# DARYL-GWZ/Proud-SLAM

Measured on AMD Instinct MI355X. Metric: rays/sec render+backward, Replica room0, 64 samples/ray, 1/2/4/8 MI355X, higher is better.
Workload: dtype f32

## Files before the change

include/psvo.h:

```cpp
#ifndef PSVO_H
#define PSVO_H

#include <stdint.h>

#ifdef __cplusplus
extern "C" {
#endif

enum {
    PSVO_OK = 0,
    PSVO_E_INVALID = 1,
    PSVO_E_LAUNCH = 2,
    PSVO_E_OVERFLOW = 3,
    PSVO_E_BUSY = 4,
    PSVO_E_SYSTEM = 5
};

const char *psvo_last_error(void);
const char *psvo_version(void);


int psvo_svo_intersect(void *stream, int b, int n, int m, float voxelsize, int n_max, const float *ray_start,
                       const float *ray_dir, const float *points, const int *children, int *idx, float *min_depth,
                       float *max_depth);
// ... 226 lines not shown
                       float *out_dirs, float *out_rgb, float *out_depth);

int64_t psvo_rows_workspace_ints(int64_t n_rows);
int psvo_rows_compact(void *stream, int64_t n_rows, int width, const float *grad, int *workspace, int *ids,
                      float *rows, int *count);
int psvo_rows_scatter_add(void *stream, int64_t n_list, int width, const int *ids, const float *rows, float *grad);
int psvo_rows_compact_flagged(void *stream, int64_t n_rows, int width, const float *grad, const uint8_t *flags,
                              int *workspace, int *ids, float *rows, int *count);
int psvo_rows_clear(void *stream, int64_t n_list, int width, const int *ids, float *grad, uint8_t *flags);
int psvo_rows_mark(void *stream, int64_t n_list, const int *ids, uint8_t *flags);
int psvo_rows_flags_from_grad(void *stream, int64_t n_rows, int width, const float *grad, uint8_t *flags);

psvo_engine *psvo_engine_new(void);
void psvo_engine_free(psvo_engine *e);
enum { PSVO_XCH_GATHER_I32 = 1, PSVO_XCH_SUM_I32 = 2, PSVO_XCH_SUM_F64 = 3, PSVO_XCH_QUERY = 0x100 };
typedef int (*psvo_exchange_fn)(void *user, int op, int64_t in_off, int64_t out_off, int64_t count, void *stream);
int64_t psvo_engine_exchange_words(int world, int64_t max_rays_global, int64_t max_rays_rank);
int psvo_engine_set_exchange(psvo_engine *e, int rank, int world, int64_t max_rays_global, int64_t max_rays_rank,
                             psvo_exchange_fn fn, void *user, int *xi32, double *xf64);

int psvo_engine_queued(psvo_engine *e);
int psvo_map_discard(psvo_engine *e);

enum { PSVO_PATH_QUERY_SPLIT = 1, PSVO_PATH_PADDED = 2, PSVO_PATH_DENSE_DECODER = 4, PSVO_PATH_INTERP_PASS = 8 };
int psvo_engine_set_paths(psvo_engine *e, int paths);

int psvo_engine_select_stats(psvo_engine *e, void *stream, int64_t *out, int reset);

int psvo_engine_gate_stream(psvo_engine *e, void *stream);

int psvo_debug_set_lookback(int mask, int spin_bound, int delay_us);
int psvo_debug_lb_helps(int64_t *out3, int reset);
int psvo_debug_set_pixel_draw(int mode);
int psvo_debug_select_samples(void *stream, int64_t r_hit, int s_max, float truncation, float max_depth,
                              const int *offsets, const int *ray_ns, const float *z_vals, int z_stride,
                              const int *rank_ray, const float *gt_depth, const float *sdf_s, const float *feat,
                              const int *leaf, const float *t, const int *ray_of, int64_t cap, int split, int *cidx,
                              int *offa, int *offb, float *feat_c, int *leaf_c, float *t_c, int *ray_of_c,
                              float *rgb_c, int *src_c, int *counts, uint64_t *desc, uint32_t tag, int *host_flag);
int64_t psvo_debug_select_granules(int64_t r_hit);
int psvo_debug_trunk_interp(void *stream, int fused, int64_t m_cap, const int *m_dev, const int *leaf, const float *t,
                            const int *ray_of, const int *ray_index, const float *rays_o, const float *rays_d,
                            const float *centres, const int *vertex_idx, const float *emb, float voxel_size,
                            const float *w1, const float *b1, const float *w2, const float *b2, const float *w3,
                            const float *b3, const float *w4, const float *b4, const float *w5, const float *b5,
                            float *images, float *sdf, float *h2, float *feat);
int psvo_debug_composite_loss(void *stream, int64_t r_hit, int s_max, float truncation, float max_depth,
                              const int *offsets, const int *ray_ns, const float *z_vals, int z_stride,
                              const int *rank_ray, const float *gt_rgb, const float *gt_depth, const float *sdf_s,
                              const float *rgb_s, const float *coef, float *workspace, float *color, float *depth,
                              float *grad_sdf_s, float *grad_rgb_s, int partials, const int *cidx);

enum { PSVO_TIME_MLP_FWD = 0, PSVO_TIME_MLP_BWD = 1, PSVO_TIME_INTERP_FWD = 2, PSVO_TIME_INTERP_BWD = 3,
       PSVO_TIME_INTERSECT = 4, PSVO_TIME_SAMPLE = 5, PSVO_TIME_POINTS = 6, PSVO_TIME_SELECT = 7,
// ... 130 lines not shown
```

proud-slam_amd/csrc/capi.cpp:

```cpp
#include <hip/hip_runtime.h>
#include <stdarg.h>
#include <stdio.h>

#include "psvo_common.h"
#include "lookback.h"

namespace psvo {

static thread_local char g_err[512] = "";
thread_local hipEvent_t g_stop_event = nullptr;
thread_local bool g_stop_share = false;
thread_local hipEvent_t g_stop_bound = nullptr;

int set_error(int code, const char *fmt, ...) {
    va_list ap;
    va_start(ap, fmt);
    vsnprintf(g_err, sizeof(g_err), fmt, ap);
    va_end(ap);
    return code;
}

int check_launch(const char *what) {
    const hipError_t e = hipGetLastError();
    if (e != hipSuccess) return set_error(PSVO_E_LAUNCH, "%s: %s", what, hipGetErrorString(e));
    return PSVO_OK;
}

static int g_lb_debug_mask = 0, g_lb_debug_bound = -1, g_lb_debug_delay = 0;
LbCtl lb_ctl(int site) {
    const bool on = (g_lb_debug_mask & site) != 0;
    return LbCtl{on && g_lb_debug_bound >= 0 ? g_lb_debug_bound : kLbSpinMax, on ? g_lb_debug_delay : 0};
}

}

extern "C" int psvo_debug_set_lookback(int mask, int spin_bound, int delay_us) {
    PSVO_REQUIRE(mask >= 0 && mask <= 7 && spin_bound >= -1 && delay_us >= 0 && delay_us <= 100000,
                 "debug_set_lookback: bad arguments");
    psvo::g_lb_debug_mask = mask;
    psvo::g_lb_debug_bound = spin_bound;
    psvo::g_lb_debug_delay = delay_us;
    return PSVO_OK;
}

extern "C" int psvo_debug_lb_helps(int64_t *out3, int reset) {
    PSVO_REQUIRE(out3, "debug_lb_helps: null argument");
    const int rc = psvo::lb_helps_query(out3, reset != 0);
    if (rc != PSVO_OK) return rc;
    return psvo::lb_helps_select(out3 + 2, reset != 0);
}

extern "C" int psvo_debug_select_samples(void *stream, int64_t r_hit, int s_max, float truncation, float max_depth,
                                         const int *offsets, const int *ray_ns, const float *z_vals, int z_stride,
                                         const int *rank_ray, const float *gt_depth, const float *sdf_s,
                                         const float *feat, const int *leaf, const float *t, const int *ray_of,
                                         int64_t cap, int split, int *cidx, int *offa, int *offb, float *feat_c,
// ... 25 lines not shown
```

proud-slam_amd/csrc/engine.cpp:

```cpp
#include <stdio.h>
#include <stdlib.h>
#include <string.h>

#include <utility>

#include "engine_internal.h"

namespace psvo {
RenderWs *&engine_render_ws(psvo_engine *e) { return e->render; }
bool engine_data_parallel(const psvo_engine *e) { return e->x.on(); }
}

using namespace psvo;
using namespace psvo::eng;

namespace psvo {
thread_local KernelClock *g_kclock = nullptr;

namespace eng {

void *arena_buf(Arena &a, hipStream_t st, int slot, size_t bytes, int *rc) {
    if (bytes == 0) bytes = 16;
    if (a.cap[slot] >= bytes) return a.p[slot];
    if (a.p[slot]) {
// ... 201 lines not shown
}

int pose_adam(hipStream_t st, const psvo_map_desc *d, const PoseAdam &pa) {
    if (pa.n == 0) return PSVO_OK;
    int64_t n6[kXchMaxFrames];
    double lr[kXchMaxFrames];
    int zero[kXchMaxFrames];
    for (int k = 0; k < pa.n; ++k) {
        n6[k] = 6;
        lr[k] = pa.lr;
        zero[k] = 0;
    }
    return adam_launch(st, pa.n, pa.p, pa.g, pa.m, pa.v, n6, lr, d->beta1, d->beta2, d->eps, 0.0, 1, zero,
                       const_cast<int64_t *>(pa.step));
}

}
}

extern "C" psvo_engine *psvo_engine_new(void) {
    psvo_engine *e = new psvo_engine();
    const char *ipass = getenv("PSVO_INTERP_PASS");
    if (ipass && ipass[0] == '1') e->paths |= PSVO_PATH_INTERP_PASS;
    for (auto &q : e->qs)
        if (query_set_init(q) != PSVO_OK) {
            psvo_engine_free(e);
            return nullptr;
        }
    return e;
}

static EngineExchange exchange_layout(int world, int64_t max_rays_global, int64_t max_rays_rank) {
    EngineExchange x;
    x.world = world;
    x.nch = dist_slot0_rows(max_rays_global) / kSamplerG;
    x.max_rays_rank = max_rays_rank > 0 ? max_rays_rank : max_rays_global;
    x.cw = dist_count_words((int)x.max_rays_rank);
    return x;
}

extern "C" int64_t psvo_engine_exchange_words(int world, int64_t max_rays_global, int64_t max_rays_rank) {
    if (world < 1 || max_rays_global < 1 || max_rays_rank < 0 || max_rays_rank > max_rays_global) return -1;
    const EngineExchange x = exchange_layout(world, max_rays_global, max_rays_rank);
    return x.table_off() + x.table_words();
}

extern "C" int psvo_engine_set_exchange(psvo_engine *e, int rank, int world, int64_t max_rays_global,
                                        int64_t max_rays_rank, psvo_exchange_fn fn, void *user, int *xi32,
                                        double *xf64) {
    PSVO_REQUIRE(e, "engine_set_exchange: null engine");
    PSVO_REQUIRE(world >= 1 && rank >= 0 && rank < world && max_rays_global >= 1 && max_rays_rank >= 0 &&
                     max_rays_rank <= max_rays_global,
                 "engine_set_exchange: bad rank %d / world %d / max_rays_global %lld / max_rays_rank %lld", rank,
                 world, (long long)max_rays_global, (long long)max_rays_rank);
    PSVO_REQUIRE(e->q_count == 0, "engine_set_exchange: queries are queued");
    PSVO_REQUIRE(!fn || (xi32 && xf64), "engine_set_exchange: exchange buffers required");
    e->x = exchange_layout(world, max_rays_global, max_rays_rank);
    e->x.fn = fn;
    e->x.user = user;
    e->x.rank = rank;
    e->x.xi32 = xi32;
    e->x.xf64 = xf64;
    return PSVO_OK;
}

extern "C" int psvo_engine_set_paths(psvo_engine *e, int paths) {
    PSVO_REQUIRE(e && (paths & ~(PSVO_PATH_QUERY_SPLIT | PSVO_PATH_PADDED | PSVO_PATH_DENSE_DECODER |
                               PSVO_PATH_INTERP_PASS)) == 0,
                 "engine_set_paths: bad arguments");
    PSVO_REQUIRE(e->q_count == 0, "engine_set_paths: queries are queued");
    e->paths = paths;
    return PSVO_OK;
}

extern "C" int psvo_engine_gate_stream(psvo_engine *e, void *stream) {
    PSVO_REQUIRE(e, "engine_gate_stream: null engine");
    e->draw_gate_used = true;
    if (!e->draw_gate_recorded) return PSVO_OK;
    return st_wait(as_stream(stream), e->draw_gate_ev, "engine_gate_stream");
}

extern "C" int psvo_engine_select_stats(psvo_engine *e, void *stream, int64_t *out, int reset) {
    PSVO_REQUIRE(e && out, "engine_select_stats: null argument");
    for (int i = 0; i < 5; ++i) out[i] = 0;
    if (!e->a.p[kSelCnt]) return PSVO_OK;
    hipStream_t st = as_stream(stream);
    int c[psvo::kSelCountInts];
    if (hipMemcpyAsync(c, e->a.p[kSelCnt], sizeof(c), hipMemcpyDeviceToHost, st) != hipSuccess ||
        hipStreamSynchronize(st) != hipSuccess)
        return set_error(PSVO_E_LAUNCH, "engine_select_stats: copy failed");
    unsigned long long u[3];
// ... 174 lines not shown
```

proud-slam_amd/csrc/engine_step.cpp:

```cpp
#include <stdint.h>
#include <string.h>

#include <algorithm>

#include "engine_internal.h"
#include "interp_load.h"

using namespace psvo;
using namespace psvo::eng;

namespace {

struct Samples {
    int *offsets = nullptr, *leaf = nullptr, *ray_of = nullptr;
    float *tt = nullptr, *feat = nullptr, *rgb_s = nullptr, *act = nullptr;
    uint64_t *masks = nullptr;
};

struct Render {
    int64_t r_hit = 0, m = 0;
    int s_max = 0;
    int *rank_ray = nullptr, *ray_rank = nullptr, *ray_ns = nullptr;
    float *z_vals = nullptr, *images = nullptr, *sdf_s = nullptr;
    Samples s;
// ... 592 lines not shown
    const Render &q = s.q;
    const Samples &k = s.k;
    int rc = PSVO_OK;
    const int64_t M = q.m, R = s.R;
    const int n_split = 256;
    ENG_BUF(float, mlp_ws, kMlpWs, psvo_mlp_workspace_floats_w(M, d->width, n_split) * sizeof(float));
    ENG_BUF(float, dfeat, kDfeat, M * 16 * sizeof(float));
    const bool fuse_ib = psvo::mlp_bwd_fuses_interp(d->width);
    float *grad_emb = s.grads;
    const size_t emb_bytes = (size_t)d->n_emb * 16 * sizeof(float);
    const bool emb_dirty = !(e->grads_clean && e->clean_buf == grad_emb);
    if (fuse_ib && emb_dirty) ENG_CALL(zero_async(grad_emb, emb_bytes, st, "map_step"));
    float *gx = nullptr;
    if (fuse_ib) {
        ENG_BUF(float, gxb, kIbWs, (size_t)s.m_rows() * 3 * sizeof(float));
        gx = gxb;
    }
    const psvo::InterpFuse ipf{k.leaf,  k.ray_of,      q.rank_ray, d->vertex_idx, k.tt, s.rays_o, s.rays_d, d->centres,
                               d->emb,  d->voxel_size, grad_emb,   gx,            s.mark_into};
    mark(e, st, PSVO_TIME_MLP_BWD, 0);
    const psvo::InterpFuse ipf_b{k.leaf + M, k.ray_of + M, q.rank_ray, d->vertex_idx, k.tt + M, s.rays_o, s.rays_d,
                                 d->centres, d->emb, d->voxel_size, grad_emb, gx ? gx + 3 * M : nullptr, s.mark_into};
    const psvo::TrunkBwd tbw{s.sel_cnt ? s.sel_cnt + 1 : nullptr, s.g_sdf_s + M, s.h2_src ? k.feat : k.feat + M * 16,
                             fuse_ib ? &ipf_b : nullptr, s.h2_src ? q.h2 : nullptr, s.h2_src ? s.h2_src + M : nullptr};
    ENG_CALL(mlp_bwd(st, M, d->width, k.feat, q.images, k.rgb_s, k.act, k.masks, s.g_sdf_s, s.g_rgb_s, dfeat, s.G, 0,
                     n_split, mlp_ws, s.overlap ? e->dfeat_ready : nullptr, fuse_ib ? &ipf : nullptr,
                     s.split ? ax : nullptr, s.sel_cnt, s.two_class() ? &tbw : nullptr, s.h2_src));
    mark(e, st, PSVO_TIME_MLP_BWD, 1);
    if (s.overlap) e->bwd_recorded = true;
    if (s.overlap && eb != st) ENG_CALL(st_wait(eb, e->dfeat_ready, "map_step"));
    if (!fuse_ib && emb_dirty) ENG_CALL(zero_async(grad_emb, emb_bytes, eb, "map_step"));
    e->grads_clean = false;
    e->clean_buf = grad_emb;
    mark(e, eb, PSVO_TIME_INTERP_BWD, 0);
    if (fuse_ib) {
        ENG_CALL(psvo::interp_rays_gx(eb, q.r_hit, k.offsets, q.rank_ray, k.tt, gx, s.grad_od, s.grad_od + R * 3,
                                      s.two_class() ? s.offb : nullptr, s.two_class() ? k.tt + M : nullptr,
                                      s.two_class() ? gx + 3 * M : nullptr));
    } else {
        ENG_BUF(float, ib_ws2, kIbWs, psvo_interp_bwd_workspace_floats(q.r_hit, q.s_max) * sizeof(float));
        ENG_CALL(psvo_interp_bwd_chunked(eb, q.r_hit, q.s_max, 16, d->voxel_size, k.offsets, q.rank_ray, k.leaf, k.tt,
                                         s.rays_o, s.rays_d, d->centres, d->vertex_idx, d->emb, dfeat, grad_emb,
                                         s.grad_od, s.grad_od + R * 3, ib_ws2));
    }
    mark(e, eb, PSVO_TIME_INTERP_BWD, 1);
    if (s.overlap && eb != st) {
        ENG_CALL(ev_record(e->emb_done, eb, "map_step"));
// ... 201 lines not shown
```

proud-slam_amd/csrc/mlp128_trunk_fb.h:

```cpp
#pragma once
#include "interp_fuse.h"
#include "mlp128_chain16.h"

namespace psvo {
namespace {

using ifuse::interp_bwd_unit;
using ifuse::scatter_unit;

constexpr int kT4H2 = kVecPad;
constexpr int kT4H1 = kT4H2 + 4 * kUImg;
constexpr int kT4CF = kT4H1 + 4 * kUImg;
constexpr int kT4X = kT4CF + 2 * kCfTile;
constexpr int kT4I = kT4X + 2 * 4 * 16 * kU;
constexpr int kT4R = kT4I + 4 * 512;
constexpr int kT4M = kT4R + 4 * 132;
constexpr int kLdsTrunk = (kT4M + 4 * 64 * 2) * 4;
static_assert(kLdsTrunk <= 160 * 1024, "trunk kernel LDS budget");

struct TrunkIn {
    float gs;
    float4 x;
    int src;
};
// ... 66 lines not shown
        for (int ob = 0; ob < 8; ++ob)
#pragma unroll
            for (int j = 0; j < 4; ++j) r0[ob][j] = row_sum16(fb[ob][j] * dsdf);
        if (n == 0) {
#pragma unroll
            for (int ob = 0; ob < 8; ++ob) {
                float4 *pp = reinterpret_cast<float4 *>(page3 + 16 * ob + 4 * q);
                const float4 o = *pp;
                *pp = make_float4(o.x + r0[ob][0], o.y + r0[ob][1], o.z + r0[ob][2], o.w + r0[ob][3]);
            }
        }
    }
    b30p += dsdf;
#pragma unroll
    for (int ob = 0; ob < 8; ++ob) {
        const float4 w = *reinterpret_cast<const float4 *>(lds + kOffW3r0 + 16 * ob + 4 * q);
        fb[ob] = f32x4v{__fmul_rn(w.x, dsdf), __fmul_rn(w.y, dsdf), __fmul_rn(w.z, dsdf), __fmul_rn(w.w, dsdf)};
    }
    mask16(fb, m2);
    lds_u_store<8>(lds + kT4H2 + k * kUImg, wb, fb);
}

template <bool H2>
__global__ __launch_bounds__(kF2Threads, 1) void k_mlp_trunk_fb(const int *__restrict__ m_dev,
                                                                const float *__restrict__ img,
                                                                const float *__restrict__ g_sdf,
                                                                const float *__restrict__ feat, DwGrid g,
                                                                float *__restrict__ slabs, InterpFuse ip,
                                                                const float *__restrict__ h2,
                                                                const int *__restrict__ h2_src) {
    extern __shared__ __attribute__((aligned(16))) float lds[];
    const int64_t m = __builtin_amdgcn_readfirstlane(*m_dev);
    const int lane = threadIdx.x & 63;
    const int wave = __builtin_amdgcn_readfirstlane(threadIdx.x >> 6);
    const int64_t n_units = (m + kU - 1) / kU;
    const int64_t u0 = n_units * blockIdx.x / gridDim.x, u1 = n_units * (blockIdx.x + 1) / gridDim.x;
    const int n_rounds = (int)((u1 - u0 + 3) / 4);
    float *const h2set = lds + kT4H2, *const h1set = lds + kT4H1, *const cf = lds + kT4CF;
    auto xset = [&](int par) { return lds + kT4X + (par & 1) * 4 * 16 * kU; };
    stage8(lds, img + kImgVec, kVecPad, wave, lane);
    wait_vm(0);
    raw_barrier();
    const int b = blockIdx.x;
    const int i = lane & 31, h = lane >> 5;
    const int n = lane & 15, q = lane >> 4;
    const int sn = (n & 1) * 8 + (n >> 1);
    const int wb = 64 * q + ((((sn >> 2) ^ q) << 2) | (sn & 3));
    const __amdgpu_buffer_rsrc_t wrs = rsrc_of(img, (int64_t)kImgTotal * 4);
    const bool fuse = ip.gx != nullptr;
    [[maybe_unused]] constexpr int kStampK = 2;
    PSVO_STAMP_DECL;
    if (wave < 4) {
        const int c = wave;
        f32x4v w1acc[8];
        zero4(w1acc);
        float b1p[8] = {0.f, 0.f, 0.f, 0.f, 0.f, 0.f, 0.f, 0.f};
        int lf_n = 0, ro_n = 0;
        float ts_n = 0.f;
        {
            const int64_t u = u0 + c;
            const int64_t s = u * kU + n;
            if (fuse && u < u1 && s < m) {
                lf_n = ip.leaf[s];
                ro_n = ip.ray_of[s];
                ts_n = ip.t[s];
            }
// ... 164 lines not shown
                for (int k = 0; k < 4; ++k) v += lds[kT4M + k * 128 + e - 128 * 16];
            }
            store_nt(s1, e, v);
        }
    }
    if (wave >= 4) {
        const int d = wave - 4;
        float *s3 = slabs + g.slab_off[2] + (int64_t)b * g.slab_len[2];
        if (h == 0) {
            float v = 0.f;
#pragma unroll
            for (int k = 0; k < 4; ++k) v += lds[kT4R + k * 132 + 32 * d + i];
            store_nt(s3, 32 * d + i, v);
        }
        if (d == 0 && lane == 0) {
            float v = 0.f;
#pragma unroll
            for (int k = 0; k < 4; ++k) v += lds[kT4R + k * 132 + 128];
            store_nt(s3, 129 * 128, v);
        }
    }
}

void launch_trunk_fb(hipStream_t st, int grid, const float *images, const TrunkBwd &tb, const DwGrid &g,
                     float *slabs) {
    const InterpFuse ip = tb.ip ? *tb.ip : InterpFuse{};
    if (tb.h2)
        launch_lds<k_mlp_trunk_fb<true>>(dim3(grid), dim3(kF2Threads), kLdsTrunk, st, tb.m_dev, images, tb.g_sdf,
                                         tb.feat, g, slabs, ip, tb.h2, tb.src);
    else
        launch_lds<k_mlp_trunk_fb<false>>(dim3(grid), dim3(kF2Threads), kLdsTrunk, st, tb.m_dev, images, tb.g_sdf,
                                          tb.feat, g, slabs, ip, tb.h2, tb.src);
}

}
}
```

proud-slam_amd/csrc/mlp_bwd.hip:

```cpp
#include <hip/hip_runtime.h>

#include <cstdlib>

#include "interp_fuse.h"
#include "mlp128_chain16.h"
#include "mlp128_trunk_fb.h"
#include "psvo_common.h"

namespace psvo {
namespace {

constexpr int kDwRedEl = 64;
__device__ __forceinline__ float dw_sum_range(const float *__restrict__ p, int64_t stride, int b, int e) {
    float v = 0.0f;
    int sp = b;
    for (; sp + 8 <= e; sp += 8) {
        float q[8];
#pragma unroll
        for (int u = 0; u < 8; ++u) q[u] = p[(sp + u) * stride];
#pragma unroll
        for (int u = 0; u < 8; ++u) v += q[u];
    }
    for (; sp < e; ++sp) v += p[sp * stride];
    return v;
}
__global__ __launch_bounds__(256) void k_mlp_dw_reduce(DwGrid g, const float *__restrict__ slabs, DwDst dst,
                                                       int accumulate, const float *__restrict__ slabs_b) {
    __shared__ float part[4][kDwRedEl];
    const int lane = threadIdx.x & 63, k = threadIdx.x >> 6;
    const int e = blockIdx.x * kDwRedEl + lane;
    const bool in = e < dst.elem_begin[5];
    int L = 0;
#pragma unroll
    for (int l = 1; l < 5; ++l) L += (e >= dst.elem_begin[l]);
    const int rel = in ? e - dst.elem_begin[L] : 0;
    const int n_split = g.n_split[L];
    const int64_t stride = g.slab_len[L];
    const int b = n_split * k / 4, en = n_split * (k + 1) / 4;
    float v = 0.0f;
    if (in) {
        v = dw_sum_range(slabs + g.slab_off[L] + rel, stride, b, en);
        if (slabs_b && (L < 2 || (L == 2 && (rel < 128 || rel == 129 * 128))))
            v += dw_sum_range(slabs_b + g.slab_off[L] + rel, stride, b, en);
    }
    part[k][lane] = v;
    __syncthreads();
    if (k != 0 || !in) return;
    v = ((part[0][lane] + part[1][lane]) + part[2][lane]) + part[3][lane];
    const int nw = dst.rows[L] * dst.cols[L];
    float *out = rel < nw ? dst.w[L] + rel : dst.b[L] + (rel - nw);
    *out = accumulate ? *out + v : v;
}

struct BwdIn16 {
    uint64_t mk[3];
    float y[3], g[3], gs;
    float4 x;
};

__device__ __forceinline__ void load_bwd_in16(const float *__restrict__ rgb_in, const uint64_t *__restrict__ masks,
                                              const float *__restrict__ g_sdf, const float *__restrict__ g_rgb,
                                              const float *__restrict__ feat, int64_t s, bool valid, int q,
                                              BwdIn16 &in, const int *__restrict__ x_src = nullptr) {
    const int64_t sv = valid ? s : 0;
    const uint64_t *mk = masks + (sv * 2 + (q & 1)) * 3;
#pragma unroll
    for (int i = 0; i < 3; ++i) {
        in.mk[i] = mk[i];
        in.y[i] = rgb_in[sv * 3 + i];
        in.g[i] = g_rgb[sv * 3 + i];
    }
    in.gs = g_sdf[sv];
    const int64_t xr = x_src ? (int64_t)x_src[sv] : sv;
    in.x = *reinterpret_cast<const float4 *>(feat + xr * kIn + 4 * q);
}

struct Bwd3Src {
    const float *rgb, *g_sdf, *g_rgb, *feat;
    const uint64_t *masks;
    const float *act;
    float *dfeat;
    const int *x_src;
};

template <bool W>
__global__ __launch_bounds__(kF2Threads, 1) void k_mlp_bwd3(int64_t m, const float *__restrict__ img, Bwd3Src src,
                                                            DwGrid g, float *__restrict__ slabs, InterpFuse ip,
                                                            const int *__restrict__ m_dev) {
    extern __shared__ __attribute__((aligned(16))) float lds[];
    if (m_dev) m = __builtin_amdgcn_readfirstlane(*m_dev);
    const int lane = threadIdx.x & 63;
    const int wave = __builtin_amdgcn_readfirstlane(threadIdx.x >> 6);
    const int64_t n_tiles = (m + kCh - 1) / kCh * 2;
    const int64_t tstride = n_tiles * kCfTile;
    const int64_t tb = tstride * 4;
    const int64_t n_units = (m + kU - 1) / kU;
    const int64_t u0 = n_units * blockIdx.x / gridDim.x, u1 = n_units * (blockIdx.x + 1) / gridDim.x;
    constexpr int kPer = W ? 4 : 8;
    const int n_rounds = (int)((u1 - u0 + kPer - 1) / kPer);
    float *const slot = lds + kB3Slot, *const small = lds + kB3Small, *const xim = lds + kB3X;
    auto dset = [&](int s) { return slot + s * 4 * kUImg; };
    auto eset = [&](int e) { return dset(((e % 2) + 2) % 2); };
    auto sset = [&](int s) { return small + s * 4 * 4 * kU; };
    auto xset = [&](int par) { return xim + par * 4 * 16 * kU; };
    stage8(lds, img + kImgVec, kVecPad, wave, lane);
    wait_vm(0);
    raw_barrier();
    const int b = blockIdx.x;
    const int i = lane & 31, h = lane >> 5;
    if (!W || wave < 4) {
        const __amdgpu_buffer_rsrc_t wrs = rsrc_of(img, (int64_t)kImgTotal * 4);
        const int c = wave;
        const int n = lane & 15, q = lane >> 4;
        const int sn = (n & 1) * 8 + (n >> 1);
        const int wb = 64 * q + ((((sn >> 2) ^ q) << 2) | (sn & 3));
        float *const page1 = lds + kB3A + c * 2048, *const page4x = page1 + 1024;
        if (W) {
#pragma unroll
            for (int k = 0; k < 8; ++k)
                *reinterpret_cast<float4 *>(page1 + (k * 64 + lane) * 4) = make_float4(0.f, 0.f, 0.f, 0.f);
        }
        float b1p = 0.f;
        BwdIn16 nin;
        {
            const int64_t u = u0 + c;
            const int64_t s = u * kU + n;
            load_bwd_in16(src.rgb, src.masks, src.g_sdf, src.g_rgb, src.feat, s, u < u1 && s < m, q, nin, src.x_src);
        }
        [[maybe_unused]] constexpr int kStampK = 1;
        PSVO_STAMP_DECL;
        for (int r = 0; r <= n_rounds; ++r) {
// ... 238 lines not shown
            store_nt(s3, 32 * d + i, vr0);
        }
        if (d == 0 && lane == 0) store_nt(s3, 129 * 128, v30);
        float *s5 = slabs + g.slab_off[4] + (int64_t)b * g.slab_len[4];
        const float4 p0 = *reinterpret_cast<const float4 *>(page5), p1 = *reinterpret_cast<const float4 *>(page5 + 4);
        const float w5[3] = {p0.x, p0.y, p0.z}, b5[3] = {p1.x, p1.y, p1.z};
        float v5[3], t5[3];
#pragma unroll
        for (int ch = 0; ch < 3; ++ch) {
            v5[ch] = w5[ch] + __shfl_xor(w5[ch], 32, 64);
            t5[ch] = b5[ch] + __shfl_xor(b5[ch], 32, 64);
        }
        if (h == 0) {
#pragma unroll
            for (int ch = 0; ch < 3; ++ch) store_nt(s5, ch * 128 + 32 * d + i, v5[ch]);
        }
        if (d == 0 && lane == 0) {
#pragma unroll
            for (int ch = 0; ch < 3; ++ch) store_nt(s5, 3 * 128 + ch, t5[ch]);
        }
    }
}

int bwd3_grid(int64_t m) {
    const int64_t rounds = (m + 4 * kU - 1) / (4 * kU);
    return persistent_grid(rounds > 0 ? rounds : 1);
}
constexpr int kDwRows[5] = {128, 128, 129, 128, 3};
constexpr int kDwCols[5] = {16, 128, 128, 144, 128};
void dw_grid_uniform(int n, DwGrid *g, int *slab_floats) {
    int off = 0;
    for (int l = 0; l < 5; ++l) {
        g->n_split[l] = n;
        g->slab_off[l] = off;
        g->slab_len[l] = kDwRows[l] * kDwCols[l] + kDwRows[l];
        off += n * g->slab_len[l];
    }
    *slab_floats = off;
}

}

int64_t dec128_workspace_floats(int64_t m) {
    DwGrid g;
    int slab;
    dw_grid_uniform(bwd3_grid(m), &g, &slab);
    return m * 3 + 2 * (int64_t)slab;
}

int dec128_bwd(hipStream_t st, int64_t m, const float *feat, const float *images, const float *rgb, const float *act,
               const uint64_t *masks, const float *g_sdf, const float *g_rgb, float *dfeat, float *const gw[5],
               float *const gb[5], int accumulate, int n_split, float *workspace, hipEvent_t dfeat_ready,
               const InterpFuse *ip, hipStream_t reduce_stream, const int *m_dev, const TrunkBwd *tb,
               const int *x_src) {
    PSVO_REQUIRE(m >= 0 && n_split > 0, "mlp_bwd: bad sizes");
    PSVO_REQUIRE(images != nullptr, "mlp_bwd: images of the training forward required");
    const bool want_w = gw[0] != nullptr;
    PSVO_REQUIRE(!want_w || act != nullptr, "mlp_bwd: weight gradients need the forward's activations");
    DwGrid g;
    int slab_floats;
    PSVO_REQUIRE(tb == nullptr || (gw[0] != nullptr && tb->m_dev && tb->g_sdf && tb->feat),
                 "mlp_bwd: the trunk backward needs the weight-gradient path and its inputs");
    float *slabs_b = nullptr;
    auto reduce = [&](float *slabs, hipStream_t rs) {
        DwDst d;
        int e = 0;
        for (int l = 0; l < 5; ++l) {
            d.w[l] = gw[l];
            d.b[l] = gb[l];
            d.rows[l] = kDwRows[l];
            d.cols[l] = kDwCols[l];
            d.elem_begin[l] = e;
            e += kDwRows[l] * kDwCols[l] + kDwRows[l];
        }
        d.elem_begin[5] = e;
        psvo::launch(k_mlp_dw_reduce, dim3(div_up(e, kDwRedEl)), dim3(256), 0, rs, g, slabs, d, accumulate,
                     static_cast<const float *>(slabs_b));
        return check_launch("mlp_dw_reduce");
    };
    Bwd3Src src{rgb, g_sdf, g_rgb, feat, masks, act, dfeat, x_src};
    if (!want_w) {
        if (m > 0) {
            launch_lds<k_mlp_bwd3<false>>(dim3(persistent_grid(div_up(div_up(m, kU), 8))), dim3(kF2Threads), kLdsBwd3,
                                          st, m, images, src, g, nullptr, InterpFuse{}, m_dev);
            const int rc = check_launch("mlp_bwd3");
            if (rc) return rc;
        }
        if (dfeat_ready && hipEventRecord(dfeat_ready, st) != hipSuccess)
            return set_error(PSVO_E_LAUNCH, "mlp_bwd: event record failed");
        return PSVO_OK;
    }
    const int grid = bwd3_grid(m);
    dw_grid_uniform(grid, &g, &slab_floats);
    float *slabs = workspace + m * 3;
    static const bool bind_env = [] {
        const char *v = getenv("PSVO_BIND_DFEAT");
        return !(v && v[0] == '0');
    }();
    const bool trunk_last = tb && m > 0;
    bool bound = false;
    const hipEvent_t bind_ev = bind_env ? dfeat_ready : nullptr;
    if (m > 0) {
        psvo::StopBind sb(trunk_last ? nullptr : bind_ev);
        launch_lds<k_mlp_bwd3<true>>(dim3(grid), dim3(kF2Threads), kLdsBwd3, st, m, images, src, g, slabs,
                                     ip ? *ip : InterpFuse{}, m_dev);
        bound = sb.consumed();
        const int rc = check_launch("mlp_bwd3");
        if (rc) return rc;
    } else if (hipMemsetAsync(slabs, 0, (size_t)slab_floats * sizeof(float), st) != hipSuccess) {
        return set_error(PSVO_E_LAUNCH, "mlp_bwd: memset failed");
    }
    if (trunk_last) {
        slabs_b = slabs + slab_floats;
        PSVO_REQUIRE(!tb->h2 || tb->src, "mlp_bwd: the trunk's h2 rows need their source index");
        psvo::StopBind sb(bind_ev);
        launch_trunk_fb(st, grid, images, *tb, g, slabs_b);
        bound = sb.consumed();
        const int rc = check_launch("mlp_trunk_fb");
        if (rc) return rc;
    }
    if (dfeat_ready && !bound && hipEventRecord(dfeat_ready, st) != hipSuccess)
        return set_error(PSVO_E_LAUNCH, "mlp_bwd: event record failed");
    if (reduce_stream && reduce_stream != st) {
        PSVO_REQUIRE(dfeat_ready != nullptr, "mlp_bwd: a separate reduce stream needs the dfeat_ready event");
        if (hipStreamWaitEvent(reduce_stream, dfeat_ready, 0) != hipSuccess)
            return set_error(PSVO_E_LAUNCH, "mlp_bwd: stream wait failed");
        return reduce(slabs, reduce_stream);
    }
    return reduce(slabs, st);
}

}
```

proud-slam_amd/csrc/psvo_common.h:

```cpp
#pragma once

#include <hip/hip_ext.h>
#include <hip/hip_runtime.h>
#include <stdint.h>

#include "../../include/psvo.h"

namespace psvo {

struct KernelClock {
    static constexpr int kMax = 192, kMaxInst = 64;
    hipEvent_t ev[kMax][2] = {};
    int region[kMax] = {};
    int n = 0;
    struct Inst {
        int region, first, last;
    } inst[kMaxInst] = {};
    int n_inst = 0;
    int stack[8] = {};
    int depth = 0;
    bool sum = false;
    bool overflow = false;
    hipStream_t streams[4] = {};
    bool owns(hipStream_t st) const {
// ... 293 lines not shown
    coef[2] = (flags & PSVO_CRIT_USE_SDF) ? (float)(2.0 * (double)(fs_w * fs_weight) / n_el) : 0.0f;
    coef[3] = (flags & PSVO_CRIT_USE_SDF) ? (float)(2.0 * (double)(sdf_w * sdf_weight) / n_el) * tr : 0.0f;
}

struct InterpFuse {
    const int *leaf, *ray_of, *rank_ray, *vertex_idx;
    const float *t, *rays_o, *rays_d, *centres, *emb;
    float voxel_size;
    float *grad_emb;
    float *gx;
    uint8_t *row_flags;
};

int interp_rays_gx(hipStream_t st, int64_t r_hit, const int *offsets, const int *ray_index, const float *t,
                   const float *gx, float *grad_o, float *grad_d, const int *offsets2 = nullptr,
                   const float *t2 = nullptr, const float *gx2 = nullptr);

struct TrunkBwd {
    const int *m_dev;
    const float *g_sdf, *feat;
    const InterpFuse *ip;
    const float *h2 = nullptr;
    const int *src = nullptr;
};
int mlp_bwd(void *stream, int64_t m, int width, const float *feat, const float *images, const float *rgb,
            const float *act, const uint64_t *masks, const float *g_sdf, const float *g_rgb, float *dfeat,
            float *const *grads, int accumulate, int n_split, float *workspace, hipEvent_t dfeat_ready,
            const InterpFuse *ip = nullptr, hipStream_t reduce_stream = nullptr, const int *m_dev = nullptr,
            const TrunkBwd *tb = nullptr,
            const int *x_src = nullptr);
bool mlp_bwd_fuses_interp(int width);
bool mlp_bwd_split_tail(int width);

int mlp_images(void *stream, int width, const float *const *dec, float *images);
struct H2Rows {
    float *out = nullptr;
    const float *rows = nullptr;
    const int *src = nullptr;
};
int mlp_fwd_prepared(void *stream, int64_t m, int width, const float *feat, float *images, float *sdf, float *rgb,
                     float *act, uint64_t *masks, const int *m_dev = nullptr,
                     const H2Rows *h2 = nullptr);
int mlp_fwd(void *stream, int64_t m, int width, const float *feat, const float *const *dec, float *images, float *sdf,
            float *rgb, float *act, uint64_t *masks);

}

// ... 5 lines not shown
```

proud-slam_amd/psvo/_lib.py:

```python
from __future__ import annotations

import ctypes
import os

import torch

PKG_ROOT = os.path.dirname(os.path.dirname(os.path.abspath(__file__)))
LIB_PATH = os.environ.get("PSVO_LIB_PATH") or os.path.join(PKG_ROOT, "lib", "libpsvo.so")

_vp, _i32, _i64, _f32, _f64, _u64 = (ctypes.c_void_p, ctypes.c_int, ctypes.c_int64, ctypes.c_float,
                                      ctypes.c_double, ctypes.c_uint64)

_SIGNATURES = {
    "psvo_last_error": (ctypes.c_char_p, []),
    "psvo_version": (ctypes.c_char_p, []),
    "psvo_svo_intersect": (_i32, [_vp, _i32, _i32, _i32, _f32, _i32] + [_vp] * 7),
    "psvo_inverse_cdf_sampling": (_i32, [_vp, _i32, _i32, _i32, _i32, _f32] + [_vp] * 9),
    "psvo_ball_intersect": (_i32, [_vp, _i32, _i32, _i32, _f32, _i32] + [_vp] * 6),
    "psvo_aabb_intersect": (_i32, [_vp, _i32, _i32, _i32, _f32, _i32] + [_vp] * 6),
    "psvo_triangle_intersect": (_i32, [_vp, _i32, _i32, _i32, _f32, _f32, _i32] + [_vp] * 6),
    "psvo_uniform_ray_sampling": (_i32, [_vp, _i32, _i32, _i32, _i32, _f32] + [_vp] * 7),
    "psvo_ray_intersect_sorted": (_i32, [_vp, _i64, _vp, _vp, _vp, _vp, _f32, _f32, _f32] + [_vp] * 6),
    "psvo_hit_rank": (_i32, [_vp, _i64, _vp, _vp, _vp]),
    "psvo_sample_rays": (_i32, [_vp, _i64, _i32, _vp, _vp, _vp, _vp, _vp, _f32, _vp, _u64, _vp, _vp, _vp, _vp,
# ... 28 lines not shown
    "psvo_rows_mark": (_i32, [_vp, _i64, _vp, _vp]),
    "psvo_rows_flags_from_grad": (_i32, [_vp, _i64, _i32, _vp, _vp]),
    "psvo_mlp_image_floats": (_i64, []),
    "psvo_mlp_image_floats_w": (_i64, [_i32]),
    "psvo_mlp_act_floats": (_i64, [_i64, _i32]),
    "psvo_mlp_mask_words": (_i64, [_i64, _i32]),
    "psvo_mlp_workspace_floats_w": (_i64, [_i64, _i32, _i32]),
    "psvo_map_grad_floats_w": (_i64, [_i64, _i32]),
    "psvo_mlp_fwd": (_i32, [_vp, _i64, _i32] + [_vp] * 16),
    "psvo_mlp_workspace_floats": (_i64, [_i64, _i32]),
    "psvo_mlp_bwd": (_i32, [_vp, _i64, _i32] + [_vp] * 28 + [_i32, _i32, _vp]),
    "psvo_criterion_workspace_floats": (_i64, [_i64]),
    "psvo_criterion_sums": (_i32, [_vp, _i64, _i32, _i32, _f32, _f32] + [_vp] * 9),
    "psvo_criterion_finalize": (_i32, [_vp, _vp, _i64, _i32, _f32, _f32, _f32, _f32, _f32, _i32, _vp]),
    "psvo_criterion_bwd": (_i32, [_vp, _i64, _i32, _f32, _f32] + [_vp] * 12),
    "psvo_adam_step": (_i32, [_vp, _i32, _vp, _vp, _vp, _vp, _vp, _f64, _f64, _f64, _f64, _f64, _i64]),
    "psvo_engine_new": (_vp, []),
    "psvo_engine_free": (None, [_vp]),
    "psvo_engine_set_timing": (_i32, [_vp, _i32]),
    "psvo_engine_set_paths": (_i32, [_vp, _i32]),
    "psvo_engine_select_stats": (_i32, [_vp, _vp, _vp, _i32]),
    "psvo_engine_gate_stream": (_i32, [_vp, _vp]),
    "psvo_debug_set_lookback": (_i32, [_i32, _i32, _i32]),
    "psvo_debug_set_pixel_draw": (_i32, [_i32]),
    "psvo_debug_lb_helps": (_i32, [_vp, _i32]),
    "psvo_debug_select_samples": (_i32, [_vp, _i64, _i32, _f32, _f32, _vp, _vp, _vp, _i32] + [_vp] * 7
                                  + [_i64, _i32] + [_vp] * 11 + [ctypes.c_uint32, _vp]),
    "psvo_debug_select_granules": (_i64, [_i64]),
    "psvo_debug_trunk_interp": (_i32, [_vp, _i32, _i64] + [_vp] * 10 + [_f32] + [_vp] * 14),
    "psvo_debug_composite_loss": (_i32, [_vp, _i64, _i32, _f32, _f32, _vp, _vp, _vp, _i32] + [_vp] * 11
                                  + [_i32, _vp]),
    "psvo_engine_queued": (_i32, [_vp]),
    "psvo_map_discard": (_i32, [_vp]),
    "psvo_engine_exchange_words": (_i64, [_i32, _i64, _i64]),
    "psvo_engine_set_exchange": (_i32, [_vp, _i32, _i32, _i64, _i64, _vp, _vp, _vp, _vp]),
    "psvo_engine_timing": (_i32, [_vp, _vp]),
    "psvo_engine_set_clock": (_i32, [_vp, _i32]),
    "psvo_engine_clock": (_i32, [_vp, _vp, _vp]),
    "psvo_host_wait_stats": (_i32, [_vp, _vp, _vp, _i32]),
    "psvo_map_step": (_i32, [_vp, _vp, _vp, _i64, _vp, _vp, _vp, _vp, _u64, _i64, _i32, _vp, _vp]),
    "psvo_map_adam": (_i32, [_vp, _vp, _vp, _i64]),
    "psvo_map_adam_ex": (_i32, [_vp, _vp, _vp, _i64, _i32]),
    "psvo_map_join": (_i32, [_vp, _vp]),
    "psvo_map_side_wait": (_i32, [_vp, _vp]),
    "psvo_engine_grad_rays": (_i32, [_vp, _vp, _i64, _vp, _vp]),
    "psvo_map_query": (_i32, [_vp, _vp, _vp, _i64, _vp, _vp, _u64]),
# ... 132 lines not shown
```

proud-slam_amd/psvo/engine.py:

```python
from __future__ import annotations

import ctypes
import os

import torch

from . import _lib as L

_vp, _i32, _i64, _f32, _f64 = ctypes.c_void_p, ctypes.c_int, ctypes.c_int64, ctypes.c_float, ctypes.c_double


class MapDesc(ctypes.Structure):
    _fields_ = [("n_nodes", _i64), ("centres", _vp), ("structure", _vp), ("vertex_idx", _vp),
                ("emb", _vp), ("n_emb", _i64), ("emb_m", _vp), ("emb_v", _vp),
                ("dec", _vp * 10), ("dec_m", _vp * 10), ("dec_v", _vp * 10), ("width", _i32),
                ("voxel_size", _f32), ("step_size", _f32), ("max_distance", _f32), ("truncation", _f32),
                ("max_depth", _f32), ("w_rgb", _f32), ("w_depth", _f32), ("w_fs", _f32), ("w_sdf", _f32),
                ("lr_emb", _f64), ("lr_dec", _f64), ("beta1", _f64), ("beta2", _f64), ("eps", _f64),
                ("grad_flat", _vp), ("packed", _vp), ("emb_row_flags", _vp), ("emb_row_local", _vp)]


class MapFrames(ctypes.Structure):
    _fields_ = [("n_frames", _i32), ("rays_per_frame", _i64), ("dirs_cam", _vp), ("poses", _vp), ("pose_m", _vp),
                ("pose_v", _vp), ("pose_step", _vp), ("lr_pose", _f64), ("pose_grad", _vp),
# ... 253 lines not shown
                                   "(pass the same tensor objects and seed)")
        else:
            ro = rays_o.reshape(-1, 3).float().contiguous()
            rd = rays_d.reshape(-1, 3).float().contiguous()
        gt_rgb = rgb.reshape(-1, 3).float().contiguous()
        gt_d = depth.reshape(-1).float().contiguous()
        self.step_no += 1
        rc = _lib().psvo_map_step(self.handle, L.stream_of(ro.device), ctypes.addressof(self.desc), ro.shape[0],
                                  ro.data_ptr(), rd.data_ptr(), gt_rgb.data_ptr(), gt_d.data_ptr(), int(seed),
                                  self.step_no, 0 if apply_adam else 1, self.loss_out.data_ptr(),
                                  ctypes.addressof(self.stats))
        self._sync_queue()
        if rc != 0:
            self.step_no -= 1
            raise self._error("psvo_map_step", rc)
        return self.loss_out[0]

    def adam(self):
        ge = self.grad_exchange
        marked = ge is not None and ge.take_rows_marked()
        L.call("psvo_map_adam_ex", self.handle, L.stream_of(self.emb.device), ctypes.addressof(self.desc),
               self.step_no, 1 if marked else 0)

    PATH_QUERY_SPLIT, PATH_PADDED, PATH_DENSE_DECODER, PATH_INTERP_PASS = 1, 2, 4, 8

    def set_paths(self, paths):
        L.call("psvo_engine_set_paths", self.handle, int(paths))

    def select_stats(self, reset=False):
        out = (ctypes.c_int64 * 5)()
        L.call("psvo_engine_select_stats", self.handle, L.stream_of(self.emb.device), ctypes.cast(out, ctypes.c_void_p),
               int(bool(reset)))
        return {"kept": out[0], "composited": out[1], "kept_sum": out[2], "composited_sum": out[3], "steps": out[4]}

    def set_timing(self, on):
        L.call("psvo_engine_set_timing", self.handle, 2 if on == "overlap" else int(bool(on)))

    def set_clock(self, max_steps):
        L.call("psvo_engine_set_clock", self.handle, int(max_steps))

    def clock(self):
        ms, n = ctypes.c_double(), ctypes.c_int()
        L.call("psvo_engine_clock", self.handle, ctypes.byref(ms), ctypes.byref(n))
        return (ms.value if ms.value >= 0 else None), n.value

    @staticmethod
    def host_wait_stats(reset=False):
# ... 124 lines not shown
```

Measured before the change: 6.323 million.

## Fuse head and trunk MLP backward into one launch with cost-balanced workgroup split

Runs the head-class bwd3 and the trunk backward in a single persistent launch. Workgroups are partitioned between the two classes by a cost model (bwd_split_na) that balances the estimated rounds of each, using device-side counts. This removes a serial kernel boundary and the tail idle time between the two launches. The dw reduce kernel is adjusted to match the new split of slabs. The trade-offs are higher LDS use per workgroup (the max of both kernels' needs) and dependence on hand-tuned cost constants. The old two-launch path stays available behind an env flag.

```diff
diff --git a/include/psvo.h b/include/psvo.h
--- a/include/psvo.h
+++ b/include/psvo.h
@@ -272,7 +272,13 @@
 int psvo_engine_queued(psvo_engine *e);
 int psvo_map_discard(psvo_engine *e);
 
-enum { PSVO_PATH_QUERY_SPLIT = 1, PSVO_PATH_PADDED = 2, PSVO_PATH_DENSE_DECODER = 4, PSVO_PATH_INTERP_PASS = 8 };
+enum {
+    PSVO_PATH_QUERY_SPLIT = 1,
+    PSVO_PATH_PADDED = 2,
+    PSVO_PATH_DENSE_DECODER = 4,
+    PSVO_PATH_INTERP_PASS = 8,
+    PSVO_PATH_BWD_TWO_LAUNCH = 16
+};
 int psvo_engine_set_paths(psvo_engine *e, int paths);
 
 int psvo_engine_select_stats(psvo_engine *e, void *stream, int64_t *out, int reset);
@@ -280,6 +286,8 @@
 int psvo_engine_gate_stream(psvo_engine *e, void *stream);
 
 int psvo_debug_set_lookback(int mask, int spin_bound, int delay_us);
+int psvo_debug_set_bwd_split(int cost_a, int cost_b, int cost_b0);
+int psvo_debug_bwd_split(int64_t units_a, int64_t units_b, int n_wg);
 int psvo_debug_lb_helps(int64_t *out3, int reset);
 int psvo_debug_set_pixel_draw(int mode);
 int psvo_debug_select_samples(void *stream, int64_t r_hit, int s_max, float truncation, float max_depth,
diff --git a/proud-slam_amd/csrc/capi.cpp b/proud-slam_amd/csrc/capi.cpp
--- a/proud-slam_amd/csrc/capi.cpp
+++ b/proud-slam_amd/csrc/capi.cpp
@@ -32,6 +32,25 @@
     return LbCtl{on && g_lb_debug_bound >= 0 ? g_lb_debug_bound : kLbSpinMax, on ? g_lb_debug_delay : 0};
 }
 
+static BwdSplitCost g_bwd_split_cost = kBwdSplitCost;
+BwdSplitCost bwd_split_cost() { return g_bwd_split_cost; }
+
+}
+
+extern "C" int psvo_debug_set_bwd_split(int cost_a, int cost_b, int cost_b0) {
+    if (cost_a == 0 && cost_b == 0 && cost_b0 == 0) {
+        psvo::g_bwd_split_cost = psvo::kBwdSplitCost;
+        return PSVO_OK;
+    }
+    PSVO_REQUIRE(cost_a >= 1 && cost_a <= 4096 && cost_b >= 1 && cost_b <= 4096 && cost_b0 >= 0 && cost_b0 <= 4096,
+                 "debug_set_bwd_split: bad arguments");
+    psvo::g_bwd_split_cost = psvo::BwdSplitCost{cost_a, cost_b, cost_b0};
+    return PSVO_OK;
+}
+
+extern "C" int psvo_debug_bwd_split(int64_t units_a, int64_t units_b, int n_wg) {
+    if (units_a < 0 || units_b < 0 || n_wg < 1) return -1;
+    return psvo::bwd_split_na(units_a, units_b, n_wg, psvo::bwd_split_cost());
 }
 
 extern "C" int psvo_debug_set_lookback(int mask, int spin_bound, int delay_us) {
diff --git a/proud-slam_amd/csrc/engine.cpp b/proud-slam_amd/csrc/engine.cpp
--- a/proud-slam_amd/csrc/engine.cpp
+++ b/proud-slam_amd/csrc/engine.cpp
@@ -247,6 +247,8 @@
     psvo_engine *e = new psvo_engine();
     const char *ipass = getenv("PSVO_INTERP_PASS");
     if (ipass && ipass[0] == '1') e->paths |= PSVO_PATH_INTERP_PASS;
+    const char *two = getenv("PSVO_BWD_TWO_LAUNCH");
+    if (two && two[0] == '1') e->paths |= PSVO_PATH_BWD_TWO_LAUNCH;
     for (auto &q : e->qs)
         if (query_set_init(q) != PSVO_OK) {
             psvo_engine_free(e);
@@ -291,7 +293,7 @@
 
 extern "C" int psvo_engine_set_paths(psvo_engine *e, int paths) {
     PSVO_REQUIRE(e && (paths & ~(PSVO_PATH_QUERY_SPLIT | PSVO_PATH_PADDED | PSVO_PATH_DENSE_DECODER |
-                               PSVO_PATH_INTERP_PASS)) == 0,
+                               PSVO_PATH_INTERP_PASS | PSVO_PATH_BWD_TWO_LAUNCH)) == 0,
                  "engine_set_paths: bad arguments");
     PSVO_REQUIRE(e->q_count == 0, "engine_set_paths: queries are queued");
     e->paths = paths;
diff --git a/proud-slam_amd/csrc/engine_step.cpp b/proud-slam_amd/csrc/engine_step.cpp
--- a/proud-slam_amd/csrc/engine_step.cpp
+++ b/proud-slam_amd/csrc/engine_step.cpp
@@ -638,7 +638,8 @@
     const psvo::InterpFuse ipf_b{k.leaf + M, k.ray_of + M, q.rank_ray, d->vertex_idx, k.tt + M, s.rays_o, s.rays_d,
                                  d->centres, d->emb, d->voxel_size, grad_emb, gx ? gx + 3 * M : nullptr, s.mark_into};
     const psvo::TrunkBwd tbw{s.sel_cnt ? s.sel_cnt + 1 : nullptr, s.g_sdf_s + M, s.h2_src ? k.feat : k.feat + M * 16,
-                             fuse_ib ? &ipf_b : nullptr, s.h2_src ? q.h2 : nullptr, s.h2_src ? s.h2_src + M : nullptr};
+                             fuse_ib ? &ipf_b : nullptr, s.h2_src ? q.h2 : nullptr, s.h2_src ? s.h2_src + M : nullptr,
+                             (e->paths & PSVO_PATH_BWD_TWO_LAUNCH) != 0};
     ENG_CALL(mlp_bwd(st, M, d->width, k.feat, q.images, k.rgb_s, k.act, k.masks, s.g_sdf_s, s.g_rgb_s, dfeat, s.G, 0,
                      n_split, mlp_ws, s.overlap ? e->dfeat_ready : nullptr, fuse_ib ? &ipf : nullptr,
                      s.split ? ax : nullptr, s.sel_cnt, s.two_class() ? &tbw : nullptr, s.h2_src));
diff --git a/proud-slam_amd/csrc/mlp128_trunk_fb.h b/proud-slam_amd/csrc/mlp128_trunk_fb.h
--- a/proud-slam_amd/csrc/mlp128_trunk_fb.h
+++ b/proud-slam_amd/csrc/mlp128_trunk_fb.h
@@ -112,26 +112,22 @@
 }
 
 template <bool H2>
-__global__ __launch_bounds__(kF2Threads, 1) void k_mlp_trunk_fb(const int *__restrict__ m_dev,
-                                                                const float *__restrict__ img,
-                                                                const float *__restrict__ g_sdf,
-                                                                const float *__restrict__ feat, DwGrid g,
-                                                                float *__restrict__ slabs, InterpFuse ip,
-                                                                const float *__restrict__ h2,
-                                                                const int *__restrict__ h2_src) {
+__device__ __forceinline__ void mlp_trunk_fb_body(const unsigned wg, const unsigned n_wg, const int b, const int64_t m,
+                                                  const float *__restrict__ img, const float *__restrict__ g_sdf,
+                                                  const float *__restrict__ feat, const DwGrid &g,
+                                                  float *__restrict__ slabs, const InterpFuse &ip,
+                                                  const float *__restrict__ h2, const int *__restrict__ h2_src) {
     extern __shared__ __attribute__((aligned(16))) float lds[];
-    const int64_t m = __builtin_amdgcn_readfirstlane(*m_dev);
     const int lane = threadIdx.x & 63;
     const int wave = __builtin_amdgcn_readfirstlane(threadIdx.x >> 6);
     const int64_t n_units = (m + kU - 1) / kU;
-    const int64_t u0 = n_units * blockIdx.x / gridDim.x, u1 = n_units * (blockIdx.x + 1) / gridDim.x;
+    const int64_t u0 = n_units * wg / n_wg, u1 = n_units * (wg + 1) / n_wg;
     const int n_rounds = (int)((u1 - u0 + 3) / 4);
     float *const h2set = lds + kT4H2, *const h1set = lds + kT4H1, *const cf = lds + kT4CF;
     auto xset = [&](int par) { return lds + kT4X + (par & 1) * 4 * 16 * kU; };
     stage8(lds, img + kImgVec, kVecPad, wave, lane);
     wait_vm(0);
     raw_barrier();
-    const int b = blockIdx.x;
     const int i = lane & 31, h = lane >> 5;
     const int n = lane & 15, q = lane >> 4;
     const int sn = (n & 1) * 8 + (n >> 1);
@@ -342,6 +338,18 @@
     }
 }
 
+template <bool H2>
+__global__ __launch_bounds__(kF2Threads, 1) void k_mlp_trunk_fb(const int *__restrict__ m_dev,
+                                                                const float *__restrict__ img,
+                                                                const float *__restrict__ g_sdf,
+                                                                const float *__restrict__ feat, DwGrid g,
+                                                                float *__restrict__ slabs, InterpFuse ip,
+                                                                const float *__restrict__ h2,
+                                                                const int *__restrict__ h2_src) {
+    const int64_t m = __builtin_amdgcn_readfirstlane(*m_dev);
+    mlp_trunk_fb_body<H2>(blockIdx.x, gridDim.x, blockIdx.x, m, img, g_sdf, feat, g, slabs, ip, h2, h2_src);
+}
+
 void launch_trunk_fb(hipStream_t st, int grid, const float *images, const TrunkBwd &tb, const DwGrid &g,
                      float *slabs) {
     const InterpFuse ip = tb.ip ? *tb.ip : InterpFuse{};
diff --git a/proud-slam_amd/csrc/mlp_bwd.hip b/proud-slam_amd/csrc/mlp_bwd.hip
--- a/proud-slam_amd/csrc/mlp_bwd.hip
+++ b/proud-slam_amd/csrc/mlp_bwd.hip
@@ -25,7 +25,9 @@
     return v;
 }
 __global__ __launch_bounds__(256) void k_mlp_dw_reduce(DwGrid g, const float *__restrict__ slabs, DwDst dst,
-                                                       int accumulate, const float *__restrict__ slabs_b) {
+                                                       int accumulate, const float *__restrict__ slabs_b,
+                                                       const int *__restrict__ cnt, const int *__restrict__ cnt_b,
+                                                       BwdSplitCost cost) {
     __shared__ float part[4][kDwRedEl];
     const int lane = threadIdx.x & 63, k = threadIdx.x >> 6;
     const int e = blockIdx.x * kDwRedEl + lane;
@@ -34,14 +36,19 @@
 #pragma unroll
     for (int l = 1; l < 5; ++l) L += (e >= dst.elem_begin[l]);
     const int rel = in ? e - dst.elem_begin[L] : 0;
-    const int n_split = g.n_split[L];
+    const bool trunk_el = L < 2 || (L == 2 && (rel < 128 || rel == 129 * 128));
+    int n_split = g.n_split[L];
+    if (cnt) {
+        const int64_t m_a = __builtin_amdgcn_readfirstlane(*cnt), m_b = __builtin_amdgcn_readfirstlane(*cnt_b);
+        const int n_a = bwd_split_na((m_a + kU - 1) / kU, (m_b + kU - 1) / kU, n_split, cost);
+        if (!trunk_el) n_split = n_a;
+    }
     const int64_t stride = g.slab_len[L];
     const int b = n_split * k / 4, en = n_split * (k + 1) / 4;
     float v = 0.0f;
     if (in) {
         v = dw_sum_range(slabs + g.slab_off[L] + rel, stride, b, en);
-        if (slabs_b && (L < 2 || (L == 2 && (rel < 128 || rel == 129 * 128))))
-            v += dw_sum_range(slabs_b + g.slab_off[L] + rel, stride, b, en);
+        if (slabs_b && trunk_el) v += dw_sum_range(slabs_b + g.slab_off[L] + rel, stride, b, en);
     }
     part[k][lane] = v;
     __syncthreads();
@@ -84,18 +91,17 @@
 };
 
 template <bool W>
-__global__ __launch_bounds__(kF2Threads, 1) void k_mlp_bwd3(int64_t m, const float *__restrict__ img, Bwd3Src src,
-                                                            DwGrid g, float *__restrict__ slabs, InterpFuse ip,
-                                                            const int *__restrict__ m_dev) {
+__device__ __forceinline__ void mlp_bwd3_body(const unsigned wg, const unsigned n_wg, const int b, const int64_t m,
+                                              const float *__restrict__ img, const Bwd3Src &src, const DwGrid &g,
+                                              float *__restrict__ slabs, const InterpFuse &ip) {
     extern __shared__ __attribute__((aligned(16))) float lds[];
-    if (m_dev) m = __builtin_amdgcn_readfirstlane(*m_dev);
     const int lane = threadIdx.x & 63;
     const int wave = __builtin_amdgcn_readfirstlane(threadIdx.x >> 6);
     const int64_t n_tiles = (m + kCh - 1) / kCh * 2;
     const int64_t tstride = n_tiles * kCfTile;
     const int64_t tb = tstride * 4;
     const int64_t n_units = (m + kU - 1) / kU;
-    const int64_t u0 = n_units * blockIdx.x / gridDim.x, u1 = n_units * (blockIdx.x + 1) / gridDim.x;
+    const int64_t u0 = n_units * wg / n_wg, u1 = n_units * (wg + 1) / n_wg;
     constexpr int kPer = W ? 4 : 8;
     const int n_rounds = (int)((u1 - u0 + kPer - 1) / kPer);
     float *const slot = lds + kB3Slot, *const small = lds + kB3Small, *const xim = lds + kB3X;
@@ -106,7 +112,6 @@
     stage8(lds, img + kImgVec, kVecPad, wave, lane);
     wait_vm(0);
     raw_barrier();
-    const int b = blockIdx.x;
     const int i = lane & 31, h = lane >> 5;
     if (!W || wave < 4) {
         const __amdgpu_buffer_rsrc_t wrs = rsrc_of(img, (int64_t)kImgTotal * 4);
@@ -391,6 +396,35 @@
     }
 }
 
+template <bool W>
+__global__ __launch_bounds__(kF2Threads, 1) void k_mlp_bwd3(int64_t m, const float *__restrict__ img, Bwd3Src src,
+                                                            DwGrid g, float *__restrict__ slabs, InterpFuse ip,
+                                                            const int *__restrict__ m_dev) {
+    if (m_dev) m = __builtin_amdgcn_readfirstlane(*m_dev);
+    mlp_bwd3_body<W>(blockIdx.x, gridDim.x, blockIdx.x, m, img, src, g, slabs, ip);
+}
+
+struct TrunkSrc {
+    const int *m_dev;
+    const float *g_sdf, *feat, *h2;
+    const int *h2_src;
+};
+template <bool W, bool H2>
+__global__ __launch_bounds__(kF2Threads, 1) void k_mlp_bwd3(int64_t m, const float *__restrict__ img, Bwd3Src src,
+                                                            DwGrid g, float *__restrict__ slabs, InterpFuse ip,
+                                                            const int *__restrict__ m_dev, TrunkSrc tk,
+                                                            InterpFuse ip_b, BwdSplitCost cost) {
+    static_assert(W, "the two-class launch is a training launch");
+    const int n_wg = gridDim.x, b = blockIdx.x;
+    if (m_dev) m = __builtin_amdgcn_readfirstlane(*m_dev);
+    const int64_t m_b = __builtin_amdgcn_readfirstlane(*tk.m_dev);
+    const int n_a = bwd_split_na((m + kU - 1) / kU, (m_b + kU - 1) / kU, n_wg, cost);
+    if (b < n_a)
+        mlp_bwd3_body<true>(b, n_a, b, m, img, src, g, slabs, ip);
+    else
+        mlp_trunk_fb_body<H2>(b - n_a, n_wg - n_a, b, m_b, img, tk.g_sdf, tk.feat, g, slabs, ip_b, tk.h2, tk.h2_src);
+}
+
 int bwd3_grid(int64_t m) {
     const int64_t rounds = (m + 4 * kU - 1) / (4 * kU);
     return persistent_grid(rounds > 0 ? rounds : 1);
@@ -431,6 +465,8 @@
     PSVO_REQUIRE(tb == nullptr || (gw[0] != nullptr && tb->m_dev && tb->g_sdf && tb->feat),
                  "mlp_bwd: the trunk backward needs the weight-gradient path and its inputs");
     float *slabs_b = nullptr;
+    const int *cnt_a = nullptr, *cnt_b = nullptr;
+    const BwdSplitCost cost = bwd_split_cost();
     auto reduce = [&](float *slabs, hipStream_t rs) {
         DwDst d;
         int e = 0;
@@ -444,7 +480,7 @@
         }
         d.elem_begin[5] = e;
         psvo::launch(k_mlp_dw_reduce, dim3(div_up(e, kDwRedEl)), dim3(256), 0, rs, g, slabs, d, accumulate,
-                     static_cast<const float *>(slabs_b));
+                     static_cast<const float *>(slabs_b), cnt_a, cnt_b, cost);
         return check_launch("mlp_dw_reduce");
     };
     Bwd3Src src{rgb, g_sdf, g_rgb, feat, masks, act, dfeat, x_src};
@@ -469,7 +505,25 @@
     const bool trunk_last = tb && m > 0;
     bool bound = false;
     const hipEvent_t bind_ev = bind_env ? dfeat_ready : nullptr;
-    if (m > 0) {
+    const bool one_launch = trunk_last && grid >= 2 && m_dev && !tb->two_launch;
+    if (one_launch) {
+        PSVO_REQUIRE(!tb->h2 || tb->src, "mlp_bwd: the trunk's h2 rows need their source index");
+        cnt_a = m_dev;
+        cnt_b = tb->m_dev;
+        const TrunkSrc tk{tb->m_dev, tb->g_sdf, tb->feat, tb->h2, tb->src};
+        const InterpFuse ip_a = ip ? *ip : InterpFuse{}, ip_b = tb->ip ? *tb->ip : InterpFuse{};
+        constexpr int kLdsAb = kLdsBwd3 > kLdsTrunk ? kLdsBwd3 : kLdsTrunk;
+        psvo::StopBind sb(bind_ev);
+        if (tb->h2)
+            launch_lds<k_mlp_bwd3<true, true>>(dim3(grid), dim3(kF2Threads), kLdsAb, st, m, images, src, g, slabs,
+                                               ip_a, m_dev, tk, ip_b, cost);
+        else
+            launch_lds<k_mlp_bwd3<true, false>>(dim3(grid), dim3(kF2Threads), kLdsAb, st, m, images, src, g, slabs,
+                                                ip_a, m_dev, tk, ip_b, cost);
+        bound = sb.consumed();
+        const int rc = check_launch("mlp_bwd3 (both classes)");
+        if (rc) return rc;
+    } else if (m > 0) {
         psvo::StopBind sb(trunk_last ? nullptr : bind_ev);
         launch_lds<k_mlp_bwd3<true>>(dim3(grid), dim3(kF2Threads), kLdsBwd3, st, m, images, src, g, slabs,
                                      ip ? *ip : InterpFuse{}, m_dev);
@@ -479,7 +533,7 @@
     } else if (hipMemsetAsync(slabs, 0, (size_t)slab_floats * sizeof(float), st) != hipSuccess) {
         return set_error(PSVO_E_LAUNCH, "mlp_bwd: memset failed");
     }
-    if (trunk_last) {
+    if (trunk_last && !one_launch) {
         slabs_b = slabs + slab_floats;
         PSVO_REQUIRE(!tb->h2 || tb->src, "mlp_bwd: the trunk's h2 rows need their source index");
         psvo::StopBind sb(bind_ev);
diff --git a/proud-slam_amd/csrc/psvo_common.h b/proud-slam_amd/csrc/psvo_common.h
--- a/proud-slam_amd/csrc/psvo_common.h
+++ b/proud-slam_amd/csrc/psvo_common.h
@@ -339,7 +339,34 @@
     const InterpFuse *ip;
     const float *h2 = nullptr;
     const int *src = nullptr;
-};
+    bool two_launch = false;
+};
+
+struct BwdSplitCost {
+    int a, b, b0;
+};
+constexpr BwdSplitCost kBwdSplitCost = {75, 35, 16};
+BwdSplitCost bwd_split_cost();
+__host__ __device__ inline int64_t bwd_split_rounds(int64_t units, int n) { return ((units + n - 1) / n + 3) / 4; }
+__host__ __device__ inline int bwd_split_na(int64_t units_a, int64_t units_b, int n_wg, BwdSplitCost c) {
+    if (units_a <= 0) return 0;
+    if (units_b <= 0 || n_wg < 2) return n_wg;
+    auto t_a = [&](int n) { return bwd_split_rounds(units_a, n) * c.a; };
+    auto t_b = [&](int n) { return bwd_split_rounds(units_b, n_wg - n) * c.b + c.b0; };
+    int lo = 1, hi = n_wg - 1;
+    while (lo < hi) {
+        const int mid = (lo + hi) / 2;
+        if (t_a(mid) <= t_b(mid))
+            hi = mid;
+        else
+            lo = mid + 1;
+    }
+    auto t = [&](int n) {
+        const int64_t ta = t_a(n), tb = t_b(n);
+        return ta > tb ? ta : tb;
+    };
+    return lo > 1 && t(lo - 1) < t(lo) ? lo - 1 : lo;
+}
 int mlp_bwd(void *stream, int64_t m, int width, const float *feat, const float *images, const float *rgb,
             const float *act, const uint64_t *masks, const float *g_sdf, const float *g_rgb, float *dfeat,
             float *const *grads, int accumulate, int n_split, float *workspace, hipEvent_t dfeat_ready,
diff --git a/proud-slam_amd/psvo/_lib.py b/proud-slam_amd/psvo/_lib.py
--- a/proud-slam_amd/psvo/_lib.py
+++ b/proud-slam_amd/psvo/_lib.py
@@ -74,6 +74,8 @@
     "psvo_engine_select_stats": (_i32, [_vp, _vp, _vp, _i32]),
     "psvo_engine_gate_stream": (_i32, [_vp, _vp]),
     "psvo_debug_set_lookback": (_i32, [_i32, _i32, _i32]),
+    "psvo_debug_set_bwd_split": (_i32, [_i32, _i32, _i32]),
+    "psvo_debug_bwd_split": (_i32, [_i64, _i64, _i32]),
     "psvo_debug_set_pixel_draw": (_i32, [_i32]),
     "psvo_debug_lb_helps": (_i32, [_vp, _i32]),
     "psvo_debug_select_samples": (_i32, [_vp, _i64, _i32, _f32, _f32, _vp, _vp, _vp, _i32] + [_vp] * 7
diff --git a/proud-slam_amd/psvo/engine.py b/proud-slam_amd/psvo/engine.py
--- a/proud-slam_amd/psvo/engine.py
+++ b/proud-slam_amd/psvo/engine.py
@@ -299,7 +299,7 @@
         L.call("psvo_map_adam_ex", self.handle, L.stream_of(self.emb.device), ctypes.addressof(self.desc),
                self.step_no, 1 if marked else 0)
 
-    PATH_QUERY_SPLIT, PATH_PADDED, PATH_DENSE_DECODER, PATH_INTERP_PASS = 1, 2, 4, 8
+    PATH_QUERY_SPLIT, PATH_PADDED, PATH_DENSE_DECODER, PATH_INTERP_PASS, PATH_BWD_TWO_LAUNCH = 1, 2, 4, 8, 16
 
     def set_paths(self, paths):
         L.call("psvo_engine_set_paths", self.handle, int(paths))
```

Measured after the change: 6.572 million, median of 6. 3.9% higher.
